# patour/distributed-membership

Measured on AMD Instinct MI355X. Metric: simulated node-ticks/sec + achieved HBM GB/s at N=65,536 full-membership, higher is better.
Workload: dtype u8 cells (u16 escape lists) / 4-bit payload (integer)

## Files before the change

distributed-membership_amd/csrc/gm_band.h:

```cpp
#pragma once
#include "gm_device.h"
#include "gm_scaled.h"

template <int B>
struct RowMeta {
  int k;
  int snd[S_SB];
  uint32_t ebase;
  uint32_t bz;
  uint64_t evc;
  uint32_t ebase2, bz2;
  uint64_t evc2;
};

template <typename T>
__device__ __forceinline__ T gld(const T *p) {
#if __HIP_DEVICE_COMPILE__
  return *(const __attribute__((address_space(1))) T *)p;
#else
  return *p;
#endif
}
template <int B, bool UNI, bool EVC = false>
__device__ __forceinline__ RowMeta<B> row_meta(const SState &s, int r, int par, int t, size_t slab, int band,
// ... 87 lines not shown
      kw[i >> 2] |= unpk(((u16x2)(1) - drop) * (u16x2)(0xFu << (4 * (3 - (i & 3)))));
    }
    return (uint64_t)kw[0] | ((uint64_t)kw[1] << 32);
  }
  uint64_t km = 0;
  for (int q = 0; q < 16; q++) {
    const uint32_t h = gm_fmix32(pair ^ ((uint32_t)((c + q) >> 1) * S_PHI));
    if (((h >> (16 * ((c + q) & 1))) & 0xFFFFu) >= T) km |= 0xFull << nib_pos(q);
  }
  return km;
}
__device__ __forceinline__ uint32_t nz_nibble_bits(uint32_t x) { return (x | (x >> 1) | (x >> 2) | (x >> 3)) & 0x11111111u; }

template <int B>
__device__ __forceinline__ void unit_table(const SState &s, UnitIn<B> &in) {
  constexpr int LPR = B / S_COLS_PER_LANE, Q = S_COLS_PER_LANE;
  const int li = (threadIdx.x & 63) % LPR;
  const __amdgpu_buffer_rsrc_t trs = gm_rsrc(s.table + (size_t)in.band * s.n * B, (uint32_t)(s.n * B));
  in.ta = __builtin_amdgcn_raw_buffer_load_b128(trs, (uint32_t)(in.r * B + li * Q), 0, GM_AUX_NT);
}

template <int B, bool UNI = false, bool EVC = false, bool TWO = false>
__device__ __forceinline__ void unit_load(const SState &s, int t, int band, int ub, UnitIn<B> &in,
                                          UnitIn<B> &in2, int band2) {
  constexpr int LPR = B / S_COLS_PER_LANE, RPW = 64 / LPR;
  const int sub = (threadIdx.x & 63) / LPR;
  in.band = band;
  in.r = ub * RPW + sub;
  in.msg = s.msg;
  in.tesc = (t & 1) ? s.tesc_in[0] : s.tesc_in[1];
  if (UNI) asm("" : "+s"(in.msg), "+s"(in.tesc));
  const size_t slab = (size_t)in.band * s.n;
  unit_table<B>(s, in);
  const RowMeta<B> meta = row_meta<B, UNI, EVC>(s, in.r, t & 1, t, slab, band, TWO ? band2 : -1);
#pragma unroll
  for (int j = 0; j < S_SB; j++) in.snd[j] = meta.snd[j];
  in.k = meta.k;
  in.ebase = meta.ebase;
  in.bz = meta.bz;
  in.evc = meta.evc;
  in.uni = EVC;
  if (TWO) {
    in2.band = band2;
    in2.r = in.r;
#pragma unroll
    for (int j = 0; j < S_SB; j++) in2.snd[j] = meta.snd[j];
    in2.k = meta.k;
    in2.ebase = meta.ebase2;
    in2.bz = meta.bz2;
    in2.evc = meta.evc2;
    in2.uni = EVC;
    in2.msg = in.msg;
    in2.tesc = in.tesc;
  }
}
template <int B, bool UNI = false, bool EVC = false>
__device__ __forceinline__ void unit_load(const SState &s, int t, int band, int ub, UnitIn<B> &in) {
  unit_load<B, UNI, EVC, false>(s, t, band, ub, in, in, -1);
}

template <int B, bool DROP>
__device__ __forceinline__ void unit_gather(const SState &s, int t, const UnitIn<B> &in, u32x2 m[S_SB], uint32_t &ent) {
  constexpr int LPR = B / S_COLS_PER_LANE;
  const int li = (threadIdx.x & 63) % LPR;
  ent = 0;
  if (li < (int)min(S_EW_TOT(in.ebase), (uint32_t)S_ESC_IN))
    ent = gld(in.tesc + ((size_t)in.band * s.n + in.r) * S_ESC_IN + li);
  const __amdgpu_buffer_rsrc_t prs = gm_rsrc(in.msg + (size_t)in.band * s.n * B, (uint32_t)(s.n * B));
  const uint32_t poff = (uint32_t)(((t & 1) ^ 1) * (B / 2) + li * 8);
  const int k = min(in.k, S_KMAX);
#pragma unroll
  for (int j = 0; j < S_SB; j++)
    m[j] = __builtin_amdgcn_raw_buffer_load_b64(prs, j < k ? poff + (uint32_t)in.snd[j] * B : GM_OOB, 0, 0);
}

struct RowCounts {
  uint64_t piece;
  int pf;
};
__device__ __forceinline__ RowCounts row_counts(int npres, int nfail) {
  int pf = npres | (nfail << 16);
  pf += __builtin_amdgcn_update_dpp(0, pf, 0xB1, 0xF, 0xF, false);
  pf += __builtin_amdgcn_update_dpp(0, pf, 0x4E, 0xF, 0xF, false);
  pf += __builtin_amdgcn_update_dpp(0, pf, 0x141, 0xF, 0xF, false);
  RowCounts rc;
  rc.piece = 0;
  rc.pf = 0;
#pragma unroll
  for (int c = 0; c < 8; c++) {
    const int v = __builtin_amdgcn_readlane(pf, 8 * c);
    rc.piece |= (uint64_t)(v & 0xFF) << (8 * c);
    rc.pf += v;
  }
  return rc;
}
template <int B, bool DROP>
__device__ __forceinline__ void unit_records(const SState &s, int t, const UnitIn<B> &in, bool live, uint32_t eb_out,
                                             int npres, int nfail, int nev, uint32_t evk, int nkept,
                                             const RowCounts *pre = nullptr) {
  constexpr int LPR = B / S_COLS_PER_LANE;
  constexpr int Q = S_COLS_PER_LANE;
  const int lane = threadIdx.x & 63;
  const int sub = lane / LPR, li = lane % LPR;
  const int band = in.band, r = in.r;
  const int colb = band * B + li * Q;
  const size_t slab = (size_t)band * s.n;
// ... 61 lines not shown
      const int q = bit >> 1;
      const uint32_t kind = (evk >> (2 * q)) & 3u;
      const uint32_t rec = (kind << 30) | (uint32_t)(s.c0 + colb + q + 1);
      if (slot < E) {
        slots[slot] = rec;
      } else {
        const uint32_t sp = sbase + (uint32_t)(slot - E);
        if (sp < s.ev_spill_cap) s.ev_spill[sp] = ((uint64_t)(uint32_t)r << 32) | rec;
        else atomicOr(s.err, GM_ERR_EVENTS);
      }
      slot++;
    }
  }
  if (li == 0 && r < s.n) {
    const uint32_t bc = (uint32_t)(pf & 0xFFFF) | ((uint32_t)(pf >> 16) << 11) | ((uint32_t)min(tot, 1023) << 22);
    s.brec[slab + r] = live ? make_uint4((uint32_t)piece, (uint32_t)(piece >> 32), bc, eb_out)
                            : make_uint4(0u, 0u, 0u, eb_out);
  }
}

template <int B, bool DROP>
__device__ __forceinline__ void unit_finish(const SState &s, int t, int drop_pct, const UnitIn<B> &in,
                                            const u32x2 m[S_SB], uint32_t ent, uint32_t *lds) {
  constexpr int LPR = B / S_COLS_PER_LANE;
  constexpr int RPW = 64 / LPR;
  constexpr int Q = S_COLS_PER_LANE;
  const int lane = threadIdx.x & 63;
  const int par = t & 1;
  const int sub = lane / LPR, li = lane % LPR;
  const int band = in.band, r = in.r;
  const int colb = band * B + li * Q;
  const size_t slab = (size_t)band * s.n;
  const __amdgpu_buffer_rsrc_t trs = gm_rsrc(s.table + slab * B, (uint32_t)(s.n * B));
  const __amdgpu_buffer_rsrc_t prs = gm_rsrc(s.msg + slab * B, (uint32_t)(s.n * B));
  const uint32_t toff = (uint32_t)(r * B + li * Q);
  const uint32_t poff = (uint32_t)((par ^ 1) * (B / 2) + li * 8);
  int k = in.k;
  if (k > S_KMAX) {
    if (li == 0) atomicOr(s.err, GM_ERR_INBOX);
    k = S_KMAX;
  }
  const bool live = k >= 0;
  const u32x4 ta = in.ta;
  struct {
    int snd[S_SB];
  } meta;
#pragma unroll
  for (int j = 0; j < S_SB; j++) meta.snd[j] = in.snd[j];
  int kw = 0;
  {
    const int kl = live ? k : 0;
#pragma unroll
    for (int w = 0; w < RPW; w++) kw = max(kw, __builtin_amdgcn_readlane(kl, w * LPR));
  }
  int npres = 0, nfail = 0, nev = 0;
  int nkept = 0;
  uint32_t evk = 0;
  bool esc_st = false;
  uint32_t eb_out = 0;
  if (!live && in.ebase != 0) {
    const int etot = (int)S_EW_TOT(in.ebase);
    eb_out = row_alloc<LPR>(s, par, slab, r, etot, li, lane);
    if (eb_out != 0) {
      const EscList src = esc_list(s, par ^ 1, slab, r, in.ebase), dst = esc_list(s, par, slab, r, eb_out);
      constexpr int P = LPR < S_ESC_IN ? LPR : S_ESC_IN;
      if (li < min(etot, P)) *dst.at(li) = ent;
      for (int i = P + li; i < etot; i += LPR) *dst.at(i) = *src.at(i);
    }
  }
  if (live) {
    const int32_t *ib = s.inbox[par] + (size_t)r * S_KMAX;
    u16x2 key5[8];
    {
      const uint32_t T = DROP ? s_drop_thresh(drop_pct) : 0u;
      const bool agrp = ((s.c0 + colb) & 1) == 0;
      u16x2 acc[8];
#pragma unroll
      for (int i = 0; i < 8; i++) acc[i] = (u16x2)(0);
      auto merge_list = [&](int sn, uint32_t x0, uint32_t x1) {
        if (DROP) {
          if (!(x0 | x1)) return;
          const uint64_t km = s_keep_nibbles(s, t, sn, r, colb, T, agrp);
          x0 &= (uint32_t)km;
          x1 &= (uint32_t)(km >> 32);
          if (s.mc_rdrop) nkept += __builtin_popcount(nz_nibble_bits(x0)) + __builtin_popcount(nz_nibble_bits(x1));
        }
        nib_max(acc, x0, x1);
      };
#pragma unroll
      for (int j = 0; j < S_SB; j++)
        if (j < kw) merge_list(meta.snd[j], m[j].x, m[j].y);
      for (int j = S_SB; j < k; j++) {
        const int sn = ib[j];
        const u32x2 mv = __builtin_amdgcn_raw_buffer_load_b64(prs, poff + (uint32_t)sn * B, 0, 0);
        merge_list(sn, mv.x, mv.y);
      }
      u16x2 nmax = (u16x2)(0);
#pragma unroll
      for (int i = 0; i < 8; i++) {
        const u16x2 nb = acc[i] >> (u16x2)(12);
        nmax = __builtin_elementwise_max(nmax, nb);
        key5[i] = pmin1(nb) * (u16x2)(S_NIB_BASE << 5) + nb * (u16x2)(64);
      }
      if (__builtin_elementwise_max(nmax.x, nmax.y) == S_NIB_ESC) {
#pragma unroll
        for (int i = 0; i < 8; i++) {
          const u16x2 nb = acc[i] >> (u16x2)(12);
#pragma unroll
          for (int h = 0; h < 2; h++) {
            if (nb[h] != S_NIB_ESC) continue;
            const int q = 2 * i + h;
            uint32_t kv = 0;
            for (int j = 0; j < k; j++) {
              const int sn = ib[j];
              if (DROP && !s_keep(s, t, sn, r, s.c0 + colb + q, T)) continue;
              const u32x2 mm = __builtin_amdgcn_raw_buffer_load_b64(prs, poff + (uint32_t)sn * B, 0, 0);
              kv = max(kv, nib_value(nib_of(mm.x, mm.y, q), s, par ^ 1, band, sn, li, q));
            }
            key5[i][h] = (uint16_t)(kv << 5);
          }
        }
      }
    }
    if (s.ramp && r == 0) {
#pragma unroll
      for (int q = 0; q < Q; q++) {
        const int c = s.c0 + colb + q;
        if (c >= 1 && colb + q < s.w && s_start(c) == t - 1) key5[q >> 1][q & 1] = (uint16_t)(255u << 5);
      }
    }
    const uint32_t tb4[4] = {ta.x, ta.y, ta.z, ta.w};
    u16x2 tw[8], npb = (u16x2)(0);
#pragma unroll
    for (int i = 0; i < 8; i++) {
      const u16x2 x = pk(byte_pair(tb4[i >> 1], i & 1));
      const u16x2 nz = pmin1(x);
      npb = padd(npb, nz);
      tw[i] = widen2(x, nz);
    }
    if (in.ebase != 0)
      esc_apply<LPR>(lds, lane, li, esc_list(s, par ^ 1, slab, r, in.ebase), (int)S_EW_TOT(in.ebase), ent, tw);
    u16x2 mm[8];
#pragma unroll
    for (int i = 0; i < 8; i++)
      mm[i] = __builtin_elementwise_max(__builtin_elementwise_sub_sat(tw[i], (u16x2)(63)), key5[i]);
    const int selfc = (r >= s.c0 && r < s.c0 + s.w) ? r - s.c0 - colb : -1;
    int selfapp = -1;
    if (selfc >= 0 && selfc < Q) {
      const int hb = s.hbctr[r] + 1;
// ... 106 lines not shown
```

distributed-membership_amd/csrc/gm_band_fast.hip:

```cpp
#include "gm_band.h"

__device__ __forceinline__ int esc_bit(int q) { return ((q & 3) << 3) | (q >> 2); }
__device__ __forceinline__ int p_lanes_below(uint64_t b) {
  return (int)__builtin_amdgcn_mbcnt_hi((uint32_t)(b >> 32), __builtin_amdgcn_mbcnt_lo((uint32_t)b, 0u));
}
struct FastCell {
  uint32_t nbyte, nib, c;
  bool gone, bail;
  int dpres, dfail;
};
__device__ __forceinline__ FastCell fast_cell(const SState &s, int t, uint32_t y, uint32_t c, bool self, int hbself) {
  FastCell o;
  if (self) {
    if (c == 0) atomicOr(s.err, GM_ERR_SELF);
    const int h = 255 - (2 * t - hbself);
    if (h < s.lag_hmin || h > 255) atomicOr(s.err, GM_ERR_LAG);
    c = (uint32_t)S_CELL(h, 0) & 0xFFFFu;
  }
  const uint32_t age = c & 31u, h = c >> 5, hp = h - 2u;
  const bool pres = c != 0, stale = pres && age >= GM_TFAIL;
  o.gone = pres && age >= GM_TREMOVE;
  const bool keep = pres && !o.gone;
  const bool fits = h >= S_H4_MIN_H && !(h & 1u) && age <= S_AGE_MAX_B;
  o.nbyte = keep ? (fits ? ((((h - 224u) >> 1) << 4) | age) : S_B_ESC) : 0u;
  const bool fresh = keep && !stale;
  const bool nibok = !(hp & 1u) && hp >= S_NIB_H(1) && hp <= S_NIB_H(14);
  o.bail = fresh && !nibok;
  o.nib = fresh && nibok ? ((hp - S_NIB_BASE) >> 1) << 4 : 0u;
  o.c = c;
  const bool fpres = y >= 16u, fstale = fpres && (y & 15u) >= GM_TFAIL;
  o.dpres = (int)(pres && !o.gone) - (int)fpres;
  o.dfail = (int)stale - (int)fstale;
  return o;
}
template <int B, typename F>
__device__ __forceinline__ bool unit_fast(const SState &s, int t, const UnitIn<B> &in, const u32x2 m[S_SB],
                                          uint32_t ent, uint32_t *lds, uint32_t *park, F &&nxt) {
  static_assert(B / S_COLS_PER_LANE == 64, "the fast path takes one row per wave");
  constexpr int Q = S_COLS_PER_LANE;
  const int lane = threadIdx.x & 63, li = lane;
  const int par = t & 1;
  const int band = in.band, r = in.r;
  const int colb = band * B + li * Q;
  const size_t slab = (size_t)band * s.n;
  const int k = in.k;
  if (k > S_KMAX || s.ramp) return false;
  if (k < 0) {
    nxt();
    uint32_t eb_out = 0;
    if (in.ebase != 0) {
      const int etot = (int)S_EW_TOT(in.ebase);
      eb_out = row_alloc<64>(s, par, slab, r, etot, li, lane);
      if (eb_out != 0) {
        const EscList src = esc_list(s, par ^ 1, slab, r, in.ebase), dst = esc_list(s, par, slab, r, eb_out);
        if (li < min(etot, S_ESC_IN)) *dst.at(li) = ent;
        for (int i = S_ESC_IN + li; i < etot; i += 64) *dst.at(i) = *src.at(i);
      }
    }
    unit_records<B, false>(s, t, in, false, eb_out, 0, 0, 0, 0u, 0);
    return true;
  }
  u16x2 acc[8];
#pragma unroll
  for (int i = 0; i < 8; i++) acc[i] = (u16x2)(0);
#pragma unroll
  for (int j = 0; j < S_SB; j++)
    if (j < k) nib_max(acc, m[j].x, m[j].y);
  if (k > S_SB) {
    const __amdgpu_buffer_rsrc_t prs = gm_rsrc(s.msg + slab * B, (uint32_t)(s.n * B));
    const uint32_t poff = (uint32_t)((par ^ 1) * (B / 2) + li * 8);
    const int32_t *ib = s.inbox[par] + (size_t)r * S_KMAX;
    for (int j = S_SB; j < k; j++) {
      const int sn = ib[j];
      const u32x2 mv = __builtin_amdgcn_raw_buffer_load_b64(prs, poff + (uint32_t)sn * B, 0, 0);
      nib_max(acc, mv.x, mv.y);
    }
  }
  {
    u16x2 amx = acc[0];
#pragma unroll
    for (int i = 1; i < 8; i++) amx = __builtin_elementwise_max(amx, acc[i]);
    if (__builtin_amdgcn_ballot_w64(__builtin_elementwise_max(amx.x, amx.y) >= (uint16_t)(S_NIB_ESC << 12)))
      return false;
  }
  const uint32_t tb4[4] = {in.ta.x, in.ta.y, in.ta.z, in.ta.w};
  uint32_t bw[4], yprev = 0;
#pragma unroll
  for (int i = 0; i < 8; i++) {
    const u16x2 x = pk(byte_pair(tb4[i >> 1], i & 1));
    const u16x2 kb = (acc[i] >> (u16x2)(8)) & (u16x2)(0xF0);
    const u16x2 y = __builtin_elementwise_max(__builtin_elementwise_sub_sat(x, (u16x2)(15)), kb);
    if (i & 1) bw[i >> 1] = __builtin_amdgcn_perm(unpk(y), yprev, 0x06040200u);
    else yprev = unpk(y);
  }
  int npres = 0, nfail = 0;
  uint32_t nb[4], spm = 0;
#pragma unroll
  for (int w = 0; w < 4; w++) {
    const uint32_t v = bw[w];
    const uint32_t lo = v & 0x0F0F0F0Fu;
    const uint32_t st = (lo + 0x01010101u * (16 - GM_TFAIL)) & 0x10101010u;
    const uint32_t a15 = (lo + 0x01010101u) & 0x10101010u;
    const uint32_t hi = v & 0xF0F0F0F0u;
    const uint32_t hs = hi >> 1;
    const uint32_t pr = (hs + 0x78787878u) & 0x80808080u;
    const uint32_t g3 = (hs + 0x68686868u) & 0x80808080u;
    nfail += __builtin_popcount(st);
    npres += __builtin_popcount(pr);
    spm |= ((pr & ~g3) | (a15 << 3)) >> (7 - w);
// ... 148 lines not shown
  const uint32_t ov0 = __builtin_amdgcn_perm(nb[1], nb[0], 0x01050004u) | (__builtin_amdgcn_perm(nb[1], nb[0], 0x03070206u) >> 4);
  const uint32_t ov1 = __builtin_amdgcn_perm(nb[3], nb[2], 0x01050004u) | (__builtin_amdgcn_perm(nb[3], nb[2], 0x03070206u) >> 4);
  int nev = 0;
  uint32_t evk = 0;
  const RowCounts rcnt = row_counts(npres, nfail);
  int tot = rcnt.pf & 0xFFFF;
  if (__builtin_amdgcn_ballot_w64(ngone != 0)) {
    int g = ngone;
    g += __builtin_amdgcn_update_dpp(0, g, 0xB1, 0xF, 0xF, false);
    g += __builtin_amdgcn_update_dpp(0, g, 0x4E, 0xF, 0xF, false);
    g += __builtin_amdgcn_update_dpp(0, g, 0x141, 0xF, 0xF, false);
    g += __builtin_amdgcn_update_dpp(0, g, 0x140, 0xF, 0xF, false);
    tot += __builtin_amdgcn_readlane(g, 0) + __builtin_amdgcn_readlane(g, 16) + __builtin_amdgcn_readlane(g, 32) +
           __builtin_amdgcn_readlane(g, 48);
  }
  if (tot != (int)S_BC_PRES(in.bz)) {
#pragma unroll
    for (int q = 0; q < Q; q++) {
      const uint32_t before = (tb4[q >> 2] >> (8 * (q & 3))) & 0xFFu;
      const uint32_t after = (bw[q >> 2] >> (8 * (q & 3))) & 0xFFu;
      const uint32_t ev = !before ? (after ? S_EV_ADD : 0u) : (!after ? S_EV_REMOVE : 0u);
      evk |= ev << (2 * q);
    }
    nev = __builtin_popcount((evk | (evk >> 1)) & 0x55555555u);
  } else if (ngone) {
    uint32_t x = gmask;
    x = (x | (x << 8)) & 0x00FF00FFu;
    x = (x | (x << 4)) & 0x0F0F0F0Fu;
    x = (x | (x << 2)) & 0x33333333u;
    x = (x | (x << 1)) & 0x55555555u;
    evk = x << 1;
    nev = ngone;
  }
  nxt();
  if (selflane) s.hbctr[r] = hbself + 1;
  uint32_t eb_out = unit_stores<B>(s, t, in, bw, ov0, ov1, false, 0u, lds);
  const uint64_t svb = __builtin_amdgcn_ballot_w64(sv);
  const bool emany = __builtin_amdgcn_ballot_w64(em != 0) != 0;
  if (svb || emany) {
    const int ns = __builtin_popcountll(svb);
    int etot = ns, eoff = 0;
    if (emany) {
      eoff = row_scan<64>(__builtin_popcount(em), li, lane, etot);
      etot += ns;
    }
    eb_out = row_alloc<64>(s, par, slab, r, etot, li, lane);
    if (eb_out != 0) {
      const EscList l = esc_list(s, par, slab, r, eb_out);
      if (sv) {
        *l.at(p_lanes_below(svb)) = sent;
        if ((sent >> 16) < (uint32_t)S_CELL(s.lag_hmin, 0)) atomicOr(s.err, GM_ERR_LAG);
      }
      if (emany) esc_emit(lds, lane, l, ns + eoff, em, li * Q, etot <= S_ESC_IN, s.err, s.lag_hmin);
    }
  }
  unit_records<B, false>(s, t, in, true, eb_out, npres, nfail, nev, evk, 0, &rcnt);
  return true;
}

#ifndef GM_FAST_WG
#define GM_FAST_WG 1
#endif
#ifndef GM_FAST_XS
#define GM_FAST_XS 8
#endif
#ifndef GM_FAST_MINW
#define GM_FAST_MINW 7
#endif
#ifndef GM_FAST_BPW
#define GM_FAST_BPW 2
#endif
template <int B, bool CH, int BPW>
__global__ __launch_bounds__(64 * GM_FAST_WG) __attribute__((amdgpu_waves_per_eu(GM_FAST_MINW, 8))) void gm_s_band_fast(SState s, int t, int u0, int u1) {
  if (!CH) {
    u0 = 0;
    u1 = s.n;
  }
  const int wv = GM_FAST_WG == 1 ? 0 : (int)(threadIdx.x >> 6);
  const uint32_t w = (uint32_t)((int)blockIdx.x * GM_FAST_WG + wv);
  const uint32_t q = (uint32_t)(u1 - u0 + GM_FAST_XS - 1) / GM_FAST_XS;
  const int ub = __builtin_amdgcn_readfirstlane(u0 + (int)((w % GM_FAST_XS) * q + w / GM_FAST_XS));
  if ((GM_FAST_WG > 1 && w / GM_FAST_XS >= q) || ub >= u1) return;
  constexpr int W = 2 * S_LDS_WAVE_WORDS + 192;
  __shared__ uint32_t lds_all[GM_FAST_WG * W];
  uint32_t *lds = lds_all + wv * W;
  const int b0 = (int)blockIdx.y * BPW;
  const bool two = BPW == 2 && b0 + 1 < s.nb;
  UnitIn<B> in, in2;
  unit_load<B, true, true, BPW == 2>(s, t, b0, ub, in, in2, two ? b0 + 1 : b0);
  u32x2 m[S_SB];
  uint32_t ent, ent2 = 0;
  unit_gather<B, false>(s, t, in, m, ent);
  bool issued = false;
  const bool ok = unit_fast<B>(s, t, in, m, ent, lds, lds + S_LDS_WAVE_WORDS, [&]() {
    if (two) {
      unit_table<B>(s, in2);
      unit_gather<B, false>(s, t, in2, m, ent2);
    }
    issued = true;
  });
  if (!ok && (threadIdx.x & 63) == 0) {
    const uint32_t slot = atomicAdd(&s.fb_cnt[t & 1], 1u);
    s.fb_list[slot] = make_int2(b0, ub);
  }
  if (two) {
    if (!issued) {
      unit_table<B>(s, in2);
      unit_gather<B, false>(s, t, in2, m, ent2);
    }
    lds_wave_sync();
    if (!unit_fast<B>(s, t, in2, m, ent2, lds, lds + S_LDS_WAVE_WORDS, []() {}) && (threadIdx.x & 63) == 0) {
      const uint32_t slot = atomicAdd(&s.fb_cnt[t & 1], 1u);
      s.fb_list[slot] = make_int2(b0 + 1, ub);
    }
  }
  if (ub == 0 && blockIdx.y == 0) band_reset_pools(s, t);
}
```

distributed-membership_amd/csrc/gm_host_scaled.hip:

```cpp
#include "gm_host.h"

using namespace gmh;

static int pick_band(const gm_ctx *c, int n, int wp) {
  int b = c->cfg.band;
  if (!b && getenv("GM_BAND")) b = atoi(getenv("GM_BAND"));
  if (b) return (b == 64 || b == 128 || b == 256 || b == 512 || b == 1024) && wp % b == 0 ? b : -1;
  const double budget = 1.4e9;
  for (int cand : {1024, 512, 256, 128})
    if (wp % cand == 0 && 5.0 * n * cand <= budget) return cand;
  return 64;
}

int gmh::create_scaled(gm_ctx *c) {
  const int n = c->n;
  const int G = c->cfg.shard_count > 0 ? c->cfg.shard_count : 1;
  const int rank = c->cfg.shard_rank;
  if (rank < 0 || rank >= G || G > n) return GM_EINVAL;
  SState &s = c->s;
  s.n = n;
  s.shard_rank = rank;
  s.shard_count = G;
  s.sharded = G > 1 || (getenv("GM_FORCE_SHARD") && atoi(getenv("GM_FORCE_SHARD")) == 1);
  auto col0 = [n, G](int g) {
    if (g >= G) return n;
    return n >= 8 * G ? 4 * (int)((int64_t)n * g / (4 * G)) : (int)((int64_t)n * g / G);
  };
  s.c0 = col0(rank);
  s.w = col0(rank + 1) - s.c0;
  s.wp = (s.w + S_ROW_ALIGN - 1) / S_ROW_ALIGN * S_ROW_ALIGN;
  s.band = pick_band(c, n, s.wp);
  if (s.band < 0) return GM_EINVAL;
  s.nb = s.wp / s.band;
  if ((size_t)n * s.band * 2 >= (1ull << 31)) return GM_EUNSUPPORTED;
  s.evs = s.band / 32;
  if (sizeof(uint32_t) * 4 * ((size_t)(s.wp / S_CHUNK(s.band)) + 1 + 624) > 65536) return GM_EUNSUPPORTED;
  s.rd_seed = c->cfg.rd_seed;
  s.drop_seed = c->cfg.drop_seed;
  const size_t cells = (size_t)n * s.wp;
  TRY(dalloc(c, &s.table, cells));
  s.kcap = inbox_cap(S_KMAX);
  s.lag_hmin = 3;
  if (getenv("GM_LAG_CAP")) {
    const int L = atoi(getenv("GM_LAG_CAP"));
    if (L < 15 || L > 125) return GM_EINVAL;
    s.lag_hmin = 254 - 2 * L;
  }
  c->shard_sync = getenv("GM_SHARD_SYNC") ? (atoi(getenv("GM_SHARD_SYNC")) ? 1 : 0) : -1;
  if (getenv("GM_DIAG_ZERO_ROW")) c->diag_zero_row = atoi(getenv("GM_DIAG_ZERO_ROW"));
  TRY(dalloc(c, &s.msg, cells));
  const size_t lists = (size_t)n * s.nb;
  int S = 1024;
  while (S > 1 && lists / S < 64) S >>= 1;
  auto grow = [&](size_t per_stripe_cells_total) {
    while ((per_stripe_cells_total + S - 1) / S > S_EW_REGION_MAX) S <<= 1;
  };
  const size_t dense_t = ((lists + 1023) / 1024) * 1024 * s.band;
  const size_t dense_p = dense_t / 16;
  const double dense_bytes = 2.0 * ((double)dense_t * 4 + (double)dense_p * 16);
  size_t free_b = 0, total_b = 0;
  HIPCHECK(hipMemGetInfo(&free_b, &total_b));
  const int gdev = c->cfg.device_share > 0 ? std::min(c->cfg.device_share, G) : G;
  double budget = (double)free_b / 4 / gdev;
  if (getenv("GM_ESC_BUDGET_GB")) budget = atof(getenv("GM_ESC_BUDGET_GB")) * 1e9;
  const bool dense = cells <= (1ull << 31) || dense_bytes <= budget;
  size_t tcells, pslots;
  if (dense) {
    while (((lists + S - 1) / S) * s.band > S_EW_REGION_MAX) S <<= 1;
    const size_t per = (lists + S - 1) / S;
    tcells = per * s.band * S;
    pslots = per * (s.band / 16) * S;
  } else {
    const double cb = (double)cells;
    double f = budget / (16.0 * cb);
    if (f > 0.25) f = (budget - 2.0 * cb) / (8.0 * cb);
    f = std::min(1.0, std::max(1.0 / 64, f));
    tcells = std::max<size_t>((size_t)(cb * f), 4 * (size_t)s.band * S);
    pslots = std::max<size_t>((size_t)(cb * std::min(1.0, 4 * f) / 16), 4 * (size_t)(s.band / 16) * S);
    grow(tcells);
  }
  s.esc_dense = dense ? 1 : 0;
  s.esc_stripes = S;
  size_t treg = std::min<size_t>((tcells + S - 1) / S, S_EW_REGION_MAX);
// ... 34 lines not shown
      !(getenv("GM_PICK0") && atoi(getenv("GM_PICK0")) == 0)) {
    TRY(dalloc(c, &s.pk_list, n));
    TRY(dalloc(c, &s.pk_cnt, 1));
  }
  TRY(dalloc(c, &s.ev_band, (size_t)n * s.nb * s.evs));
  {
    HIPCHECK(hipMemGetInfo(&free_b, &total_b));
    const size_t want = std::min<size_t>((size_t)n * s.wp, free_b / 32 / gdev / sizeof(uint64_t));
    s.ev_spill_cap = (uint32_t)std::min<size_t>(std::max<size_t>(want, 1u << 24), 1ull << 31);
  }
  TRY(dalloc(c, &s.ev_spill, s.ev_spill_cap));
  TRY(dalloc(c, &s.ev_spill_cnt, 1 + S_EV_STRIPES));
  TRY(dalloc(c, &s.evcum, (size_t)n * s.nb));
  TRY(dalloc(c, &s.mtraw, (size_t)n * S_MT_RAW));
  TRY(dalloc(c, &s.rowstat, (size_t)n * 4));
  TRY(dalloc(c, &s.targets, (size_t)n * GM_FANOUT));
  TRY(dalloc(c, &s.err, 1));
  const bool warm = c->cfg.init_mode == 1;
  const int t0 = warm ? c->cfg.init_t0 : 0;
  const bool ramp = c->cfg.init_mode == 2;
  if (c->cfg.init_mode < 0 || c->cfg.init_mode > 2 || (warm && (t0 < 5 || t0 > GM_T_LIMIT / 2))) return GM_EINVAL;
  if (ramp)
    for (int g = 1; g < G; g++)
      if (col0(g) % 4 != 0) return GM_EUNSUPPORTED;
  s.ramp = ramp ? 1 : 0;
  s.intro_until = 0x7FFFFFFF;
  if (ramp) {
    TRY(dalloc(c, &s.mecol, n));
    HIPCHECK(ctx_memset(c, s.mecol, 0xFF, sizeof(int32_t) * n));
    TRY(dalloc(c, &s.selfadd, S_SELFADD_CAP));
    TRY(dalloc(c, &s.selfadd_cnt, 1));
    HIPCHECK(ctx_memset(c, s.selfadd_cnt, 0, sizeof(uint32_t)));
  }
  HIPCHECK(ctx_memset(c, s.msg, 0, sizeof(uint8_t) * cells));
  for (int p = 0; p < 2; p++) HIPCHECK(ctx_memset(c, s.inbox_cnt[p], 0, sizeof(int32_t) * n));
  HIPCHECK(ctx_memset(c, s.failed, 0, sizeof(int32_t) * n));
  HIPCHECK(ctx_memset(c, s.err, 0, sizeof(uint32_t)));
  HIPCHECK(gm_launch_init(s, ramp ? 2 : warm ? 1 : 0, t0, c->cfg.init_seed, c->stream));
  HIPCHECK(hipStreamSynchronize(c->stream));
  uint32_t ierr = 0;
  HIPCHECK(ctx_memcpy(c, &ierr, s.err, sizeof ierr, hipMemcpyDeviceToHost));
  if (ierr) {
    snprintf(g_errbuf, sizeof g_errbuf, "initial state overflows the escape pool (%zu cells)", s.tesc_cap);
    return GM_ERANGE;
  }
  HIPCHECK(ctx_memset(c, s.ev_spill_cnt, 0, (1 + S_EV_STRIPES) * sizeof(uint32_t)));
  HIPCHECK(ctx_memset(c, s.evcum, 0, sizeof(uint64_t) * (size_t)n * s.nb));
  HIPCHECK(ctx_memset(c, s.rowstat, 0, sizeof(int32_t) * n * 4));
  if (s.sharded) {
    TRY(dalloc(c, &s.acc, (size_t)n * 8));
    TRY(dalloc(c, &s.pending, n));
    TRY(dalloc(c, &s.npending, 4));
    s.plist_cnt[1] = (uint32_t *)(s.npending + 1);
    s.plist_cnt[2] = (uint32_t *)(s.npending + 2);
    c->dmax = 64;
    {
      int K = getenv("GM_SCHUNKS") ? atoi(getenv("GM_SCHUNKS")) : 2;
      if (K < 1 || K > 64) return GM_EINVAL;
      s.xlog = 6;
      while (((int64_t)1 << s.xlog) * K < n) s.xlog++;
      s.xk = (int)((n + (1 << s.xlog) - 1) >> s.xlog);
    }
    TRY(dalloc(c, &s.xcnt, (size_t)s.xk * G * ((size_t)1 << s.xlog) * 2));
    TRY(dalloc(c, &s.status, (size_t)n * c->dmax));
    s.plist_cap[1] = std::min(S_PLIST_CAP, std::max(std::min(n, 1024), n / 16));
    s.plist_cap[2] = 256;
    if (getenv("GM_PLIST_CAP"))
// ... 60 lines not shown
```

distributed-membership_amd/csrc/gm_scaled.h:

```cpp
#pragma once
#include <stdint.h>

#include <type_traits>

#include "gm_abi.h"
#include "gm_device.h"

#define S_KMAX 64
#define S_COLS_PER_LANE 16
#define S_ROW_ALIGN 512
#define S_CHUNK(B) ((B) >= 1024 ? 128 : 64)
#define S_SB 8
#define S_MT_RAW 16
#define S_SELFADD_CAP 65536
#define S_PLIST_CAP 4096
#define S_FB_BLOCKS 2048
#define GM_D_MORE_ROUND 64
#define GM_D_LAST_ROUND 256

#define S_CELL(h, age) (((h) << 5) | (age))
#define S_B_ESC 1u
#define S_H4_MIN_H 230u
#define S_AGE_MAX_B 14u
#define S_ESC_IN 16
// ... 317 lines not shown
    if (i & 1) bw[i >> 1] = __builtin_amdgcn_perm(unpk(b), bprev, 0x06040200u);
    else bprev = unpk(b);
  }
}

template <int LPR>
__device__ __forceinline__ void payload_escapes(const SState &s, int par, size_t slab, int r, int li, int lane,
                                                int sub, bool pesc, const uint32_t cw[8]) {
  const uint64_t bal = __builtin_amdgcn_ballot_w64(pesc);
  const uint64_t rm = LPR == 64 ? bal : (bal >> (sub * LPR)) & ((1ull << LPR) - 1);
  uint32_t pbase = S_PESC_NONE;
  if (li == 0) {
    const int ps = esc_stripe(s, slab, r);
    const unsigned long long b = atomicAdd(s.pesc_cnt + par * s.esc_stripes + ps, (unsigned long long)__builtin_popcountll(rm));
    if (b + (unsigned long long)__builtin_popcountll(rm) <= (unsigned long long)s.pesc_region)
      pbase = (uint32_t)ps * s.pesc_region + (uint32_t)b;
    else atomicOr(s.err, GM_ERR_ESC);
    s.pesc_rec[par][slab + r] = make_uint4(pbase, (uint32_t)rm, (uint32_t)(rm >> 32), 0u);
  }
  pbase = LPR == 64 ? __builtin_amdgcn_readfirstlane(pbase) : (uint32_t)__shfl((int)pbase, lane - li, 64);
  uint32_t pw[8];
#pragma unroll
  for (int i = 0; i < 8; i++) {
    const u16x2 v = pk(cw[i]);
    const u16x2 stale = ((v & (u16x2)(31)) + (u16x2)(32 - GM_TFAIL)) >> (u16x2)(5);
    pw[i] = unpk(__builtin_elementwise_sub_sat(v >> (u16x2)(5), stale * (u16x2)(255) + (u16x2)(2)));
  }
  const u32x4 wv = {__builtin_amdgcn_perm(pw[1], pw[0], 0x06040200u), __builtin_amdgcn_perm(pw[3], pw[2], 0x06040200u),
                    __builtin_amdgcn_perm(pw[5], pw[4], 0x06040200u), __builtin_amdgcn_perm(pw[7], pw[6], 0x06040200u)};
  if (pesc && pbase != S_PESC_NONE)
    *(u32x4 *)(s.pesc[par] + ((size_t)pbase + __builtin_popcountll(rm & ((1ull << li) - 1))) * 16) = wv;
}

template <int B>
__device__ __forceinline__ uint32_t unit_stores(const SState &s, int t, const UnitIn<B> &in, const uint32_t bw[4],
                                                uint32_t ov0, uint32_t ov1, bool esc_row, uint32_t em, uint32_t *lds) {
  constexpr int LPR = B / S_COLS_PER_LANE;
  constexpr int Q = S_COLS_PER_LANE;
  const int lane = threadIdx.x & 63;
  const int par = t & 1;
  const int li = lane % LPR;
  const int band = in.band, r = in.r;
  const size_t slab = (size_t)band * s.n;
  const __amdgpu_buffer_rsrc_t trs = gm_rsrc(s.table + slab * B, (uint32_t)(s.n * B));
  const __amdgpu_buffer_rsrc_t prs = gm_rsrc(s.msg + slab * B, (uint32_t)(s.n * B));
  const uint32_t toff = (uint32_t)(r * B + li * Q);
  uint32_t eb_out = 0;
  const u32x4 nb4 = {bw[0], bw[1], bw[2], bw[3]};
  __builtin_amdgcn_raw_buffer_store_b128(nb4, trs, toff, 0, GM_AUX_NT);
  const u32x2 ov = {ov0, ov1};
  __builtin_amdgcn_raw_buffer_store_b64(ov, prs, (uint32_t)(r * B + par * (B / 2) + li * 8), 0, GM_AUX_NT);
  if (band == 0 && li == 0) s.wtick[r] = t;
  if (esc_row) {
    int etot;
    const int eoff = row_scan<LPR>(__builtin_popcount(em), li, lane, etot);
    eb_out = row_alloc<LPR>(s, par, slab, r, etot, li, lane);
    if (eb_out != 0) esc_emit(lds, lane, esc_list(s, par, slab, r, eb_out), eoff, em, li * Q, etot <= S_ESC_IN, s.err, s.lag_hmin);
  }
  return eb_out;
}

template <typename F>
inline hipError_t gm_band_dispatch(int band, F &&f) {
  switch (band) {
    case 64: return f(std::integral_constant<int, 64>{});
    case 128: return f(std::integral_constant<int, 128>{});
    case 256: return f(std::integral_constant<int, 256>{});
    case 512: return f(std::integral_constant<int, 512>{});
    case 1024: return f(std::integral_constant<int, 1024>{});
    default: return hipErrorInvalidValue;
  }
}

hipError_t gm_launch_tick(const SState &s, int t, int drop_pct, hipStream_t st, hipEvent_t k0, hipEvent_t k1,
                          bool pick);
hipError_t gm_launch_tick_prologue(const SState &s, int t, hipStream_t st, bool zero_draw = false);
hipError_t gm_launch_band_rows(const SState &s, int t, int drop_pct, int r0, int r1, hipStream_t st);
hipError_t gm_launch_xrows(const SState &s, int r0, int r1, hipStream_t st);
hipError_t gm_launch_draw0(const SState &s, int t, int r0, int r1, hipStream_t st);
hipError_t gm_launch_draw(const SState &s, int t, int round, int D, int listed, hipStream_t st, int r0 = 0, int r1 = -1);
hipError_t gm_launch_accept(const SState &s, int t, int D, int in_list, int out, hipStream_t st, int r0 = 0,
                            int r1 = -1);
hipError_t gm_launch_plist_sort(const SState &s, int l, hipStream_t st);
hipError_t gm_launch_init(const SState &s, int warm, int t0, uint64_t seed, hipStream_t st);
// ... 15 lines not shown
```

distributed-membership_amd/csrc/gm_scaled.hip:

```cpp
#include "gm_band.h"
#include "gm_device.h"
#include "gm_scaled.h"
#include "gm_select.h"

#include <algorithm>

__global__ __launch_bounds__(256) void gm_s_mtgen(SState s, int t, int zero_draw) {
  const int r = blockIdx.x * blockDim.x + threadIdx.x;
  if (r < 1 + S_EV_STRIPES) s.ev_spill_cnt[r] = 0;
  if (r == 0 && s.pk_cnt) *s.pk_cnt = 0;
  if (zero_draw && r == 0) {
    *s.plist_cnt[1] = 0;
    *s.plist_cnt[2] = 0;
    *s.npending = 0;
  }
  if (r >= s.n) return;
  uint32_t out[S_MT_RAW];
  gm_mt_first16(gm_rd_seed(s.rd_seed, t, r + 1), out);
  uint4 *dst = (uint4 *)(s.mtraw + (size_t)r * S_MT_RAW);
#pragma unroll
  for (int k = 0; k < S_MT_RAW / 4; k++) dst[k] = make_uint4(out[4 * k], out[4 * k + 1], out[4 * k + 2], out[4 * k + 3]);
}

hipError_t gm_launch_tick_prologue(const SState &s, int t, hipStream_t st, bool zero_draw) {
  hipLaunchKernelGGL(gm_s_mtgen, dim3((std::max(s.n, 1 + S_EV_STRIPES) + 255) / 256), dim3(256), 0, st, s, t,
                     zero_draw ? 1 : 0);
  return hipGetLastError();
}

__device__ __forceinline__ uint32_t nz_nibbles(uint32_t x) {
  return (uint32_t)__builtin_popcount((x | (x >> 1) | (x >> 2) | (x >> 3)) & 0x11111111u);
}
template <int B>
__global__ __launch_bounds__(256) void gm_s_mcfresh(SState s, int t) {
  const int lane = threadIdx.x & 63;
  const int r = blockIdx.x * 4 + (threadIdx.x >> 6);
  if (r >= s.n) return;
  const int par = t & 1, half = B / 2, tot = s.nb * half;
  uint32_t f = 0;
  for (int off = lane * 16; off < tot; off += 64 * 16) {
    const int b = off / half, o = off % half;
    const uint4 v = *(const uint4 *)(s.msg + ((size_t)b * s.n + r) * B + par * half + o);
    f += nz_nibbles(v.x) + nz_nibbles(v.y) + nz_nibbles(v.z) + nz_nibbles(v.w);
  }
#pragma unroll
  for (int o = 32; o >= 1; o >>= 1) f += __shfl_xor(f, o, 64);
  if (lane == 0) s.mc_fresh[(size_t)par * s.n + r] = f;
}

__global__ __launch_bounds__(256) void gm_s_mcount(SState s, int t, int dropped) {
  const int r = blockIdx.x * blockDim.x + threadIdx.x;
  if (r >= s.n) return;
  const int par = t & 1;
  const int32_t *stat = s.rowstat + (size_t)r * 4;
  uint32_t recv = 0;
  if (dropped) {
    recv = s.mc_rdrop[r];
    s.mc_rdrop[r] = 0;
  } else {
    const int k = min(stat[0], S_KMAX);
    for (int q = 0; q < k; q++) recv += s.mc_fresh[(size_t)(par ^ 1) * s.n + s.inbox[par][(size_t)r * S_KMAX + q]];
  }
  s.mc_sent[(size_t)t * s.n + r] = (uint32_t)stat[3] * s.mc_fresh[(size_t)par * s.n + r];
  s.mc_recv[(size_t)t * s.n + r] = recv;
}

hipError_t gm_launch_msgcount(const SState &s, int t, bool dropped, int phase, hipStream_t st) {
  if (phase == 1) {
    hipLaunchKernelGGL(gm_s_mcount, dim3((s.n + 255) / 256), dim3(256), 0, st, s, t, dropped ? 1 : 0);
    return hipGetLastError();
  }
  const dim3 g((s.n + 3) / 4), bk(256);
  return gm_band_dispatch(s.band, [&](auto b) {
    hipLaunchKernelGGL(gm_s_mcfresh<decltype(b)::value>, g, bk, 0, st, s, t);
    return hipGetLastError();
// ... 79 lines not shown
```

Baseline: 22.36 million.

## Interleave payload of band pairs so fast path gathers both bands in one load

Changes the message payload layout so two adjacent bands share a row slab, interleaved in 8-byte chunks, so one 128-bit buffer load fetches a sender's payload for both bands. The fast kernel now merges both bands' inboxes in one pass (pair_merge) and writes both outputs with a single 128-bit store instead of two 64-bit ones. The aim is fewer gather instructions and better use of each memory transaction in the HBM-bound inbox gather. The cost is more address arithmetic, a new layout every consumer (slow path, msgcount) must follow, and more registers held by two accumulator sets.

Measured after the change: 22.27 million. About the same (-0.4%).

```diff
diff --git a/distributed-membership_amd/csrc/gm_band.h b/distributed-membership_amd/csrc/gm_band.h
--- a/distributed-membership_amd/csrc/gm_band.h
+++ b/distributed-membership_amd/csrc/gm_band.h
@@ -143,6 +143,11 @@
   if (UNI) asm("" : "+s"(in.msg), "+s"(in.tesc));
   const size_t slab = (size_t)in.band * s.n;
   unit_table<B>(s, in);
+  if (TWO) {
+    in2.band = band2;
+    in2.r = in.r;
+    unit_table<B>(s, in2);
+  }
   const RowMeta<B> meta = row_meta<B, UNI, EVC>(s, in.r, t & 1, t, slab, band, TWO ? band2 : -1);
 #pragma unroll
   for (int j = 0; j < S_SB; j++) in.snd[j] = meta.snd[j];
@@ -152,8 +157,6 @@
   in.evc = meta.evc;
   in.uni = EVC;
   if (TWO) {
-    in2.band = band2;
-    in2.r = in.r;
 #pragma unroll
     for (int j = 0; j < S_SB; j++) in2.snd[j] = meta.snd[j];
     in2.k = meta.k;
@@ -177,12 +180,29 @@
   ent = 0;
   if (li < (int)min(S_EW_TOT(in.ebase), (uint32_t)S_ESC_IN))
     ent = gld(in.tesc + ((size_t)in.band * s.n + in.r) * S_ESC_IN + li);
-  const __amdgpu_buffer_rsrc_t prs = gm_rsrc(in.msg + (size_t)in.band * s.n * B, (uint32_t)(s.n * B));
-  const uint32_t poff = (uint32_t)(((t & 1) ^ 1) * (B / 2) + li * 8);
+  const __amdgpu_buffer_rsrc_t prs = pay_rsrc<B>(s, in.msg, in.band);
+  const uint32_t poff = pay_at<B>(s, in.band, 0, (t & 1) ^ 1, li * 8).off;
   const int k = min(in.k, S_KMAX);
 #pragma unroll
   for (int j = 0; j < S_SB; j++)
-    m[j] = __builtin_amdgcn_raw_buffer_load_b64(prs, j < k ? poff + (uint32_t)in.snd[j] * B : GM_OOB, 0, 0);
+    m[j] = __builtin_amdgcn_raw_buffer_load_b64(prs, j < k ? poff + (uint32_t)in.snd[j] * S_PAY_ROW(B) : GM_OOB, 0, 0);
+}
+template <int B>
+__device__ __forceinline__ void unit_gather2(const SState &s, int t, const UnitIn<B> &in, const UnitIn<B> &in2,
+                                             u32x4 m[S_SB], uint32_t &ent, uint32_t &ent2) {
+  static_assert(B / S_COLS_PER_LANE == 64, "one row per wave");
+  const int li = threadIdx.x & 63;
+  ent = ent2 = 0;
+  if (li < (int)min(S_EW_TOT(in.ebase), (uint32_t)S_ESC_IN))
+    ent = gld(in.tesc + ((size_t)in.band * s.n + in.r) * S_ESC_IN + li);
+  if (li < (int)min(S_EW_TOT(in2.ebase), (uint32_t)S_ESC_IN))
+    ent2 = gld(in.tesc + ((size_t)in2.band * s.n + in.r) * S_ESC_IN + li);
+  const __amdgpu_buffer_rsrc_t prs = pay_rsrc<B>(s, in.msg, in.band);
+  const uint32_t poff = pay_at<B>(s, in.band, 0, (t & 1) ^ 1, li * 8).off;
+  const int k = min(in.k, S_KMAX);
+#pragma unroll
+  for (int j = 0; j < S_SB; j++)
+    m[j] = __builtin_amdgcn_raw_buffer_load_b128(prs, j < k ? poff + (uint32_t)in.snd[j] * S_PAY_ROW(B) : GM_OOB, 0, 0);
 }
 
 struct RowCounts {
@@ -310,9 +330,9 @@
   const int colb = band * B + li * Q;
   const size_t slab = (size_t)band * s.n;
   const __amdgpu_buffer_rsrc_t trs = gm_rsrc(s.table + slab * B, (uint32_t)(s.n * B));
-  const __amdgpu_buffer_rsrc_t prs = gm_rsrc(s.msg + slab * B, (uint32_t)(s.n * B));
+  const __amdgpu_buffer_rsrc_t prs = pay_rsrc<B>(s, s.msg, band);
   const uint32_t toff = (uint32_t)(r * B + li * Q);
-  const uint32_t poff = (uint32_t)((par ^ 1) * (B / 2) + li * 8);
+  auto poff = [&](int sn) { return pay_at<B>(s, band, sn, par ^ 1, li * 8).off; };
   int k = in.k;
   if (k > S_KMAX) {
     if (li == 0) atomicOr(s.err, GM_ERR_INBOX);
@@ -370,7 +390,7 @@
         if (j < kw) merge_list(meta.snd[j], m[j].x, m[j].y);
       for (int j = S_SB; j < k; j++) {
         const int sn = ib[j];
-        const u32x2 mv = __builtin_amdgcn_raw_buffer_load_b64(prs, poff + (uint32_t)sn * B, 0, 0);
+        const u32x2 mv = __builtin_amdgcn_raw_buffer_load_b64(prs, poff(sn), 0, 0);
         merge_list(sn, mv.x, mv.y);
       }
       u16x2 nmax = (u16x2)(0);
@@ -392,7 +412,7 @@
             for (int j = 0; j < k; j++) {
               const int sn = ib[j];
               if (DROP && !s_keep(s, t, sn, r, s.c0 + colb + q, T)) continue;
-              const u32x2 mm = __builtin_amdgcn_raw_buffer_load_b64(prs, poff + (uint32_t)sn * B, 0, 0);
+              const u32x2 mm = __builtin_amdgcn_raw_buffer_load_b64(prs, poff(sn), 0, 0);
               kv = max(kv, nib_value(nib_of(mm.x, mm.y, q), s, par ^ 1, band, sn, li, q));
             }
             key5[i][h] = (uint16_t)(kv << 5);
diff --git a/distributed-membership_amd/csrc/gm_band_fast.hip b/distributed-membership_amd/csrc/gm_band_fast.hip
--- a/distributed-membership_amd/csrc/gm_band_fast.hip
+++ b/distributed-membership_amd/csrc/gm_band_fast.hip
@@ -33,9 +33,9 @@
   o.dfail = (int)stale - (int)fstale;
   return o;
 }
-template <int B, typename F>
-__device__ __forceinline__ bool unit_fast(const SState &s, int t, const UnitIn<B> &in, const u32x2 m[S_SB],
-                                          uint32_t ent, uint32_t *lds, uint32_t *park, F &&nxt) {
+template <int B>
+__device__ __forceinline__ bool unit_fast(const SState &s, int t, const UnitIn<B> &in, const u16x2 acc[8],
+                                          uint32_t ent, uint32_t *lds, uint32_t *park, u32x2 &ov) {
   static_assert(B / S_COLS_PER_LANE == 64, "the fast path takes one row per wave");
   constexpr int Q = S_COLS_PER_LANE;
   const int lane = threadIdx.x & 63, li = lane;
@@ -46,7 +46,6 @@
   const int k = in.k;
   if (k > S_KMAX || s.ramp) return false;
   if (k < 0) {
-    nxt();
     uint32_t eb_out = 0;
     if (in.ebase != 0) {
       const int etot = (int)S_EW_TOT(in.ebase);
@@ -59,22 +58,6 @@
     }
     unit_records<B, false>(s, t, in, false, eb_out, 0, 0, 0, 0u, 0);
     return true;
-  }
-  u16x2 acc[8];
-#pragma unroll
-  for (int i = 0; i < 8; i++) acc[i] = (u16x2)(0);
-#pragma unroll
-  for (int j = 0; j < S_SB; j++)
-    if (j < k) nib_max(acc, m[j].x, m[j].y);
-  if (k > S_SB) {
-    const __amdgpu_buffer_rsrc_t prs = gm_rsrc(s.msg + slab * B, (uint32_t)(s.n * B));
-    const uint32_t poff = (uint32_t)((par ^ 1) * (B / 2) + li * 8);
-    const int32_t *ib = s.inbox[par] + (size_t)r * S_KMAX;
-    for (int j = S_SB; j < k; j++) {
-      const int sn = ib[j];
-      const u32x2 mv = __builtin_amdgcn_raw_buffer_load_b64(prs, poff + (uint32_t)sn * B, 0, 0);
-      nib_max(acc, mv.x, mv.y);
-    }
   }
   {
     u16x2 amx = acc[0];
@@ -289,9 +272,9 @@
     evk = x << 1;
     nev = ngone;
   }
-  nxt();
   if (selflane) s.hbctr[r] = hbself + 1;
-  uint32_t eb_out = unit_stores<B>(s, t, in, bw, ov0, ov1, false, 0u, lds);
+  ov = (u32x2){ov0, ov1};
+  uint32_t eb_out = unit_stores<B>(s, t, in, bw, ov0, ov1, false, 0u, lds, false);
   const uint64_t svb = __builtin_amdgcn_ballot_w64(sv);
   const bool emany = __builtin_amdgcn_ballot_w64(em != 0) != 0;
   if (svb || emany) {
@@ -313,6 +296,45 @@
   }
   unit_records<B, false>(s, t, in, true, eb_out, npres, nfail, nev, evk, 0, &rcnt);
   return true;
+}
+
+template <int B, bool TWO>
+__device__ __forceinline__ void pair_merge(const SState &s, int t, const UnitIn<B> &in, const UnitIn<B> &in2,
+                                           u16x2 acc1[8], u16x2 acc2[8], uint32_t &ent, uint32_t &ent2) {
+  const int li = threadIdx.x & 63;
+  const int k = in.k;
+#pragma unroll
+  for (int i = 0; i < 8; i++) acc1[i] = acc2[i] = (u16x2)(0);
+  typename std::conditional<TWO, u32x4, u32x2>::type m[S_SB];
+  if constexpr (TWO) {
+    unit_gather2<B>(s, t, in, in2, m, ent, ent2);
+  } else {
+    unit_gather<B, false>(s, t, in, m, ent);
+    ent2 = 0;
+  }
+#pragma unroll
+  for (int j = 0; j < S_SB; j++)
+    if (j < k) {
+      nib_max(acc1, m[j].x, m[j].y);
+      if constexpr (TWO) nib_max(acc2, m[j].z, m[j].w);
+    }
+  if (k > S_SB) {
+    const __amdgpu_buffer_rsrc_t prs = pay_rsrc<B>(s, s.msg, in.band);
+    const int32_t *ib = s.inbox[t & 1] + (size_t)in.r * S_KMAX;
+    const int ke = min(k, S_KMAX);
+    const uint32_t poff = pay_at<B>(s, in.band, 0, (t & 1) ^ 1, li * 8).off;
+    for (int j = S_SB; j < ke; j++) {
+      const uint32_t off = poff + (uint32_t)ib[j] * S_PAY_ROW(B);
+      if constexpr (TWO) {
+        const u32x4 mv = __builtin_amdgcn_raw_buffer_load_b128(prs, off, 0, 0);
+        nib_max(acc1, mv.x, mv.y);
+        nib_max(acc2, mv.z, mv.w);
+      } else {
+        const u32x2 mv = __builtin_amdgcn_raw_buffer_load_b64(prs, off, 0, 0);
+        nib_max(acc1, mv.x, mv.y);
+      }
+    }
+  }
 }
 
 #ifndef GM_FAST_WG
@@ -345,31 +367,37 @@
   const bool two = BPW == 2 && b0 + 1 < s.nb;
   UnitIn<B> in, in2;
   unit_load<B, true, true, BPW == 2>(s, t, b0, ub, in, in2, two ? b0 + 1 : b0);
-  u32x2 m[S_SB];
-  uint32_t ent, ent2 = 0;
-  unit_gather<B, false>(s, t, in, m, ent);
-  bool issued = false;
-  const bool ok = unit_fast<B>(s, t, in, m, ent, lds, lds + S_LDS_WAVE_WORDS, [&]() {
-    if (two) {
-      unit_table<B>(s, in2);
-      unit_gather<B, false>(s, t, in2, m, ent2);
-    }
-    issued = true;
-  });
-  if (!ok && (threadIdx.x & 63) == 0) {
+  u16x2 acc1[8], acc2[8];
+  uint32_t ent, ent2;
+  if (two) pair_merge<B, true>(s, t, in, in2, acc1, acc2, ent, ent2);
+  else pair_merge<B, false>(s, t, in, in2, acc1, acc2, ent, ent2);
+  const int li = threadIdx.x & 63;
+  const bool merged = in.k >= 0;
+  u32x2 ov1 = {0u, 0u}, ov2 = {0u, 0u};
+  const bool ok1 = unit_fast<B>(s, t, in, acc1, ent, lds, lds + S_LDS_WAVE_WORDS, ov1);
+  if (!ok1 && li == 0) {
     const uint32_t slot = atomicAdd(&s.fb_cnt[t & 1], 1u);
     s.fb_list[slot] = make_int2(b0, ub);
   }
+  bool ok2 = false;
   if (two) {
-    if (!issued) {
-      unit_table<B>(s, in2);
-      unit_gather<B, false>(s, t, in2, m, ent2);
-    }
     lds_wave_sync();
-    if (!unit_fast<B>(s, t, in2, m, ent2, lds, lds + S_LDS_WAVE_WORDS, []() {}) && (threadIdx.x & 63) == 0) {
+    ok2 = unit_fast<B>(s, t, in2, acc2, ent2, lds, lds + S_LDS_WAVE_WORDS, ov2);
+    if (!ok2 && li == 0) {
       const uint32_t slot = atomicAdd(&s.fb_cnt[t & 1], 1u);
       s.fb_list[slot] = make_int2(b0 + 1, ub);
     }
   }
+  if (merged && (ok1 || ok2)) {
+    const __amdgpu_buffer_rsrc_t prs = pay_rsrc<B>(s, s.msg, b0);
+    if (ok1 && ok2) {
+      const u32x4 ov = {ov1.x, ov1.y, ov2.x, ov2.y};
+      __builtin_amdgcn_raw_buffer_store_b128(ov, prs, pay_at<B>(s, b0, ub, t & 1, li * 8).off, 0, GM_AUX_NT);
+    } else if (ok1) {
+      __builtin_amdgcn_raw_buffer_store_b64(ov1, prs, pay_at<B>(s, b0, ub, t & 1, li * 8).off, 0, GM_AUX_NT);
+    } else {
+      __builtin_amdgcn_raw_buffer_store_b64(ov2, prs, pay_at<B>(s, b0 + 1, ub, t & 1, li * 8).off, 0, GM_AUX_NT);
+    }
+  }
   if (ub == 0 && blockIdx.y == 0) band_reset_pools(s, t);
 }
diff --git a/distributed-membership_amd/csrc/gm_host_scaled.hip b/distributed-membership_amd/csrc/gm_host_scaled.hip
--- a/distributed-membership_amd/csrc/gm_host_scaled.hip
+++ b/distributed-membership_amd/csrc/gm_host_scaled.hip
@@ -48,7 +48,8 @@
   }
   c->shard_sync = getenv("GM_SHARD_SYNC") ? (atoi(getenv("GM_SHARD_SYNC")) ? 1 : 0) : -1;
   if (getenv("GM_DIAG_ZERO_ROW")) c->diag_zero_row = atoi(getenv("GM_DIAG_ZERO_ROW"));
-  TRY(dalloc(c, &s.msg, cells));
+  const size_t msg_bytes = (size_t)((s.nb + 1) / 2) * n * 2 * s.band;
+  TRY(dalloc(c, &s.msg, msg_bytes));
   const size_t lists = (size_t)n * s.nb;
   int S = 1024;
   while (S > 1 && lists / S < 64) S >>= 1;
@@ -149,7 +150,7 @@
     TRY(dalloc(c, &s.selfadd_cnt, 1));
     HIPCHECK(ctx_memset(c, s.selfadd_cnt, 0, sizeof(uint32_t)));
   }
-  HIPCHECK(ctx_memset(c, s.msg, 0, sizeof(uint8_t) * cells));
+  HIPCHECK(ctx_memset(c, s.msg, 0, msg_bytes));
   for (int p = 0; p < 2; p++) HIPCHECK(ctx_memset(c, s.inbox_cnt[p], 0, sizeof(int32_t) * n));
   HIPCHECK(ctx_memset(c, s.failed, 0, sizeof(int32_t) * n));
   HIPCHECK(ctx_memset(c, s.err, 0, sizeof(uint32_t)));
diff --git a/distributed-membership_amd/csrc/gm_scaled.h b/distributed-membership_amd/csrc/gm_scaled.h
--- a/distributed-membership_amd/csrc/gm_scaled.h
+++ b/distributed-membership_amd/csrc/gm_scaled.h
@@ -373,9 +373,27 @@
     *(u32x4 *)(s.pesc[par] + ((size_t)pbase + __builtin_popcountll(rm & ((1ull << li) - 1))) * 16) = wv;
 }
 
+#define S_PAY_ROW(B) (2u * (B))
+struct PayAt {
+  size_t slab;
+  uint32_t off;
+};
+template <int B>
+__device__ __forceinline__ PayAt pay_at(const SState &s, int band, int r, int par, uint32_t o) {
+  PayAt a;
+  a.slab = (size_t)(band >> 1) * (size_t)s.n * S_PAY_ROW(B);
+  a.off = (uint32_t)r * S_PAY_ROW(B) + (uint32_t)par * B + (o >> 3) * 16 + (uint32_t)(band & 1) * 8 + (o & 7);
+  return a;
+}
+template <int B>
+__device__ __forceinline__ __amdgpu_buffer_rsrc_t pay_rsrc(const SState &s, const uint8_t *msg, int band) {
+  return gm_rsrc(msg + pay_at<B>(s, band, 0, 0, 0).slab, (uint32_t)s.n * S_PAY_ROW(B));
+}
+
 template <int B>
 __device__ __forceinline__ uint32_t unit_stores(const SState &s, int t, const UnitIn<B> &in, const uint32_t bw[4],
-                                                uint32_t ov0, uint32_t ov1, bool esc_row, uint32_t em, uint32_t *lds) {
+                                                uint32_t ov0, uint32_t ov1, bool esc_row, uint32_t em, uint32_t *lds,
+                                                bool pay = true) {
   constexpr int LPR = B / S_COLS_PER_LANE;
   constexpr int Q = S_COLS_PER_LANE;
   const int lane = threadIdx.x & 63;
@@ -384,13 +402,15 @@
   const int band = in.band, r = in.r;
   const size_t slab = (size_t)band * s.n;
   const __amdgpu_buffer_rsrc_t trs = gm_rsrc(s.table + slab * B, (uint32_t)(s.n * B));
-  const __amdgpu_buffer_rsrc_t prs = gm_rsrc(s.msg + slab * B, (uint32_t)(s.n * B));
   const uint32_t toff = (uint32_t)(r * B + li * Q);
   uint32_t eb_out = 0;
   const u32x4 nb4 = {bw[0], bw[1], bw[2], bw[3]};
   __builtin_amdgcn_raw_buffer_store_b128(nb4, trs, toff, 0, GM_AUX_NT);
-  const u32x2 ov = {ov0, ov1};
-  __builtin_amdgcn_raw_buffer_store_b64(ov, prs, (uint32_t)(r * B + par * (B / 2) + li * 8), 0, GM_AUX_NT);
+  if (pay) {
+    const u32x2 ov = {ov0, ov1};
+    __builtin_amdgcn_raw_buffer_store_b64(ov, pay_rsrc<B>(s, s.msg, band), pay_at<B>(s, band, r, par, li * 8).off, 0,
+                                          GM_AUX_NT);
+  }
   if (band == 0 && li == 0) s.wtick[r] = t;
   if (esc_row) {
     int etot;
diff --git a/distributed-membership_amd/csrc/gm_scaled.hip b/distributed-membership_amd/csrc/gm_scaled.hip
--- a/distributed-membership_amd/csrc/gm_scaled.hip
+++ b/distributed-membership_amd/csrc/gm_scaled.hip
@@ -36,11 +36,11 @@
   const int lane = threadIdx.x & 63;
   const int r = blockIdx.x * 4 + (threadIdx.x >> 6);
   if (r >= s.n) return;
-  const int par = t & 1, half = B / 2, tot = s.nb * half;
+  const int par = t & 1, tot = ((s.nb + 1) / 2) * B;
   uint32_t f = 0;
   for (int off = lane * 16; off < tot; off += 64 * 16) {
-    const int b = off / half, o = off % half;
-    const uint4 v = *(const uint4 *)(s.msg + ((size_t)b * s.n + r) * B + par * half + o);
+    const PayAt a = pay_at<B>(s, 2 * (off / B), r, par, 0);
+    const uint4 v = *(const uint4 *)(s.msg + a.slab + a.off + off % B);
     f += nz_nibbles(v.x) + nz_nibbles(v.y) + nz_nibbles(v.z) + nz_nibbles(v.w);
   }
 #pragma unroll
```
